# kivicode/TensorHive-Fixed

Hardware: AMD Instinct MI355X
Metric: llama3_8b_bf16_ddp_train_tokens_per_sec (higher is better)
Workload: dtype bf16; 1 GPU; model=Llama-3-8B, global_batch=8, micro_batch=8, grad_accum=1, seq_len=4096, parallelism=dp1, optimizer=AdamW (fp32 master, fused flat kernel, clip 1.0), zero=0, attention=hip, gemm_table=True, gemm_table_kind=gemm_gfx950_t32768.csv

## Files before the change

tensorhive_fixed_amd/models/llama3.py:

```python
from __future__ import annotations

import math
import os
from dataclasses import dataclass

import torch
from torch import nn

from ..ops.attention import qkv_attention
from ..ops.cross_entropy import linear_cross_entropy
from ..ops.embedding import embedding
from ..ops.linear import linear
from ..ops.mlp import gate_up_swiglu
from ..ops.rmsnorm import rmsnorm, rmsnorm_add_fork, rmsnorm_fork
from ..ops.swiglu import swiglu


@dataclass
class LlamaConfig:
    vocab_size: int = 128256
    dim: int = 4096
    n_layers: int = 32
    n_heads: int = 32
    n_kv_heads: int = 8
    ffn_dim: int = 14336
    rope_theta: float = 500000.0
    norm_eps: float = 1e-5
    max_seq_len: int = 8192
    ce_chunk: int = 4096

    @property
    def head_dim(self) -> int:
        return self.dim // self.n_heads

    @classmethod
    def llama3_8b(cls) -> "LlamaConfig":
        return cls(ce_chunk=int(os.environ.get("TH_CE_CHUNK", "4096")))

    @classmethod
    def tiny(cls) -> "LlamaConfig":
        return cls(vocab_size=512, dim=256, n_layers=2, n_heads=2, n_kv_heads=1, ffn_dim=512,
                   max_seq_len=512, ce_chunk=64)

    @classmethod
    def named(cls, name: str) -> "LlamaConfig":
        table = {"llama3-8b": cls.llama3_8b, "llama3_8b": cls.llama3_8b, "tiny": cls.tiny,
                 "llama3-1b-shape": lambda: cls(dim=2048, n_layers=16, n_heads=16, n_kv_heads=4,
                                                ffn_dim=8192)}
        return table[name.lower()]()

    def num_params(self) -> int:
        d, f, v, L = self.dim, self.ffn_dim, self.vocab_size, self.n_layers
        kv = self.n_kv_heads * self.head_dim
        per_layer = d * (d + 2 * kv) + d * d + 2 * f * d + f * d + 2 * d
        return v * d * 2 + L * per_layer + d

    def flops_per_token(self, seq_len: int) -> float:
        n_mat = self.num_params() - self.vocab_size * self.dim
        attn = 2 * 2 * self.n_layers * seq_len * self.dim / 2
        return 6 * n_mat + 3 * attn


WGRAD_NT = set(filter(None, os.environ.get("TH_WGRAD_NT_LAYERS", "w13").split(",")))
WGRAD_TN = set(filter(None, os.environ.get("TH_WGRAD_TN_LAYERS", "wqkv,wo,w2").split(",")))
_FORK = os.environ.get("TH_RMSNORM_FORK", "1") == "1"


ADD_NORM = _FORK and os.environ.get("TH_ADD_NORM", "1") == "1"


def _norm(x, w, eps):
    if _FORK:
        return rmsnorm_fork(x, w, eps)
    return rmsnorm(x, w, eps), x


class LlamaBlock(nn.Module):
    def __init__(self, cfg: LlamaConfig, device, dtype):
        super().__init__()
        d, hd = cfg.dim, cfg.head_dim
        qkv_out = (cfg.n_heads + 2 * cfg.n_kv_heads) * hd
        self.cfg = cfg
        self.attn_norm = nn.Parameter(torch.ones(d, device=device, dtype=dtype))
        self.wqkv = nn.Parameter(torch.empty(qkv_out, d, device=device, dtype=dtype))
        self.wo = nn.Parameter(torch.empty(d, cfg.n_heads * hd, device=device, dtype=dtype))
        self.ffn_norm = nn.Parameter(torch.ones(d, device=device, dtype=dtype))
        self.w13 = nn.Parameter(torch.empty(2 * cfg.ffn_dim, d, device=device, dtype=dtype))
        self.w2 = nn.Parameter(torch.empty(d, cfg.ffn_dim, device=device, dtype=dtype))

    def forward(self, x: torch.Tensor, B: int, S: int, pending: torch.Tensor | None = None):
        c = self.cfg
        if pending is not None:
            h, x = rmsnorm_add_fork(pending, x, self.attn_norm, c.norm_eps)
        else:
            h, x = _norm(x, self.attn_norm, c.norm_eps)
        qkv = linear(h, self.wqkv, wgrad_nt="wqkv" in WGRAD_NT, wgrad_tn="wqkv" in WGRAD_TN)
        o = qkv_attention(qkv, B, S, c.n_heads, c.n_kv_heads, c.head_dim, c.rope_theta)
        if ADD_NORM:
            y = linear(o, self.wo, wgrad_nt="wo" in WGRAD_NT, wgrad_tn="wo" in WGRAD_TN)
            h, x = rmsnorm_add_fork(y, x, self.ffn_norm, c.norm_eps)
        else:
            x = linear(o, self.wo, residual=x, wgrad_nt="wo" in WGRAD_NT, wgrad_tn="wo" in WGRAD_TN)
            h, x = _norm(x, self.ffn_norm, c.norm_eps)
        if "w13" in WGRAD_NT:
            a = gate_up_swiglu(h, self.w13)
        else:
            a = swiglu(linear(h, self.w13))
        if ADD_NORM:
            return linear(a, self.w2, wgrad_nt="w2" in WGRAD_NT, wgrad_tn="w2" in WGRAD_TN), x
        return linear(a, self.w2, residual=x, wgrad_nt="w2" in WGRAD_NT, wgrad_tn="w2" in WGRAD_TN)


class Llama(nn.Module):
    def __init__(self, cfg: LlamaConfig, device="cpu", dtype=torch.bfloat16, seed: int = 0):
        super().__init__()
        self.cfg = cfg
        self.tok_emb = nn.Parameter(torch.empty(cfg.vocab_size, cfg.dim, device=device, dtype=dtype))
        self.layers = nn.ModuleList([LlamaBlock(cfg, device, dtype) for _ in range(cfg.n_layers)])
        self.norm = nn.Parameter(torch.ones(cfg.dim, device=device, dtype=dtype))
        self.lm_head = nn.Parameter(torch.empty(cfg.vocab_size, cfg.dim, device=device, dtype=dtype))
        self.param_gate = None
        self.reset_parameters(seed)

    @torch.no_grad()
    def reset_parameters(self, seed: int = 0) -> None:
        g = torch.Generator(device=self.tok_emb.device)
        g.manual_seed(seed)
        std = 0.02
        out_std = std / math.sqrt(2 * self.cfg.n_layers)
        self.tok_emb.normal_(0, std, generator=g)
        self.lm_head.normal_(0, std, generator=g)
        for blk in self.layers:
            blk.wqkv.normal_(0, std, generator=g)
            blk.w13.normal_(0, std, generator=g)
            blk.wo.normal_(0, out_std, generator=g)
            blk.w2.normal_(0, out_std, generator=g)

    def params_in_backward_order(self) -> list[tuple[str, nn.Parameter, bool]]:
        out = [("lm_head", self.lm_head, True), ("norm", self.norm, False)]
        for i in reversed(range(len(self.layers))):
            b = self.layers[i]
            out += [(f"layers.{i}.w2", b.w2, True), (f"layers.{i}.w13", b.w13, True),
                    (f"layers.{i}.ffn_norm", b.ffn_norm, False), (f"layers.{i}.wo", b.wo, True),
                    (f"layers.{i}.wqkv", b.wqkv, True), (f"layers.{i}.attn_norm", b.attn_norm, False)]
        out.append(("tok_emb", self.tok_emb, True))
        return out

    def hidden(self, tokens: torch.Tensor) -> torch.Tensor:
        B, S = tokens.shape
        gate = self.param_gate
        if gate is not None:
            gate(self.tok_emb)
        x = embedding(tokens, self.tok_emb).view(B * S, self.cfg.dim)
        pending = None
        for blk in self.layers:
            if gate is not None:
                gate(blk.attn_norm, blk.wqkv, blk.wo, blk.ffn_norm, blk.w13, blk.w2)
            if ADD_NORM:
                pending, x = blk(x, B, S, pending)
            else:
                x = blk(x, B, S)
        if gate is not None:
            gate(self.norm, self.lm_head)
        if pending is not None:
            return rmsnorm_add_fork(pending, x, self.norm, self.cfg.norm_eps)[0]
        return rmsnorm(x, self.norm, self.cfg.norm_eps)

    def forward(self, tokens: torch.Tensor, targets: torch.Tensor | None = None,
                n_valid: int | None = None) -> torch.Tensor:
        h = self.hidden(tokens)
        if targets is None:
            return h
        return linear_cross_entropy(h, self.lm_head, targets.reshape(-1), self.cfg.ce_chunk,
                                    n_valid=n_valid)

    @torch.no_grad()
    def logits(self, tokens: torch.Tensor) -> torch.Tensor:
        return torch.mm(self.hidden(tokens), self.lm_head.t()).view(*tokens.shape, -1)
```

tensorhive_fixed_amd/ops/_lib.py:

```python
from __future__ import annotations

import ctypes as C
import os
import threading
from pathlib import Path

import torch

_HERE = Path(__file__).resolve().parent
_LIB_PATH = Path(os.environ.get("TH_KERNEL_LIB", _HERE / "libthk.so"))
_lock = threading.Lock()
_lib: C.CDLL | None = None

P = C.c_void_p
I = C.c_int
L = C.c_long
F = C.c_float

_SIGS: dict[str, list] = {
    "th_rmsnorm_fwd": [P, P, P, P, I, I, F, P],
    "th_rmsnorm_add_fwd": [P, P, P, P, P, P, I, I, F, P],
    "th_rmsnorm_bwd": [P, P, P, P, P, P, P, I, I, I, I, P, P],
    "th_swiglu_fwd": [P, P, L, I, P],
    "th_swiglu_bwd": [P, P, P, L, I, P],
    "th_swiglu_bwd_t": [P, P, P, P, L, I, P],
    "th_rope_inplace": [P, P, P, L, I, I, I, I, F, P],
    "th_sumsq_bf16": [P, L, P, P, I, P],
    "th_adamw_step": [P, P, P, P, P, L, F, F, F, F, F, I, F, P, F, P],
    "th_adamw_step_f32g": [P, P, P, P, P, L, F, F, F, F, F, I, F, P, F, P],
    "th_sumsq_f32": [P, L, P, P, I, P],
    "th_ce_fwd_bwd": [P, L, P, P, P, L, I, F, I, P],
    "th_flash_attn_fwd": [P, P, P, P, P, I, I, I, I, I, I, L, L, L, L, F, I, P],
    "th_flash_attn_bwd": [P, P, P, P, P, P, P, P, P, P, P, I, I, I, I, I, I, L, L, L, L, F, I, P],
    "th_flash_attn_bwd_rope": [P, P, P, P, P, P, P, P, P, P, I, I, I, I, I, I, L, L, L, L, F, P, P, I, P],
    "th_embedding_bwd": [P, P, P, P, L, I, I, P],
    "th_transpose_bf16": [P, P, L, L, L, I, P],
    "th_gemm_tn": [P, L, P, L, P, L, I, I, I, I, I, I, P, L, I, P],
    "th_comm_emu_launch": [P, P, L, L, L, L, P, I, L, I, P, P],
    "th_comm_emu_stop": [P, I, P],
}


def library_path() -> Path:
    return _LIB_PATH


def load(build_if_missing: bool = False) -> C.CDLL:
    global _lib
    if _lib is not None:
        return _lib
    with _lock:
        if _lib is not None:
            return _lib
        if not _LIB_PATH.exists() and build_if_missing:
            from . import build as _build

            _build.build()
        if not _LIB_PATH.exists():
            raise RuntimeError(
                f"gfx950 kernel library {_LIB_PATH} is missing: run "
                "`python -m tensorhive_fixed_amd.ops.build` (no eager fallback on GPU)")
        if "TH_KERNEL_LIB" not in os.environ:
            from . import build as _build

            if _build.stamp_exists() and not _build.is_up_to_date():
                if build_if_missing:
                    _build.build()
                else:
                    raise RuntimeError(f"{_LIB_PATH} was built from different sources than ops/csrc: rebuild "
                                       "with `python -m tensorhive_fixed_amd.ops.build`")
        lib = C.CDLL(str(_LIB_PATH))
        for name, argtypes in _SIGS.items():
            fn = getattr(lib, name, None)
            if fn is None:
                continue
            fn.argtypes = argtypes
            fn.restype = C.c_int
        _lib = lib
        return lib


def available() -> bool:
    try:
        load()
        return True
    except (RuntimeError, OSError):
        return False


def stream_ptr(device: torch.device | None = None) -> int:
    return torch.cuda.current_stream(device).cuda_stream


def ptr(t: torch.Tensor | None) -> int | None:
    return None if t is None else t.data_ptr()


def call(name: str, *args) -> None:
    fn = getattr(load(), name, None)
    if fn is None:
        raise RuntimeError(f"kernel entry point {name} not present in {_LIB_PATH}")
    rc = fn(*args)
    if rc != 0:
        raise RuntimeError(f"{name} failed with code {rc} ({'bad shape' if rc < 0 else 'hipError'})")
```

tensorhive_fixed_amd/ops/csrc/swiglu.hip:

```cpp
#include "th_common.h"

__device__ __forceinline__ float sigmoidf_(float g) { return 1.f / (1.f + __expf(-g)); }

__global__ __launch_bounds__(256) void swiglu_fwd_kernel(const ushort* __restrict__ gu,
                                                         ushort* __restrict__ out, long T, int F) {
  const int cpr = F >> 3;
  for (long row = blockIdx.x; row < T; row += gridDim.x) {
    const ushort* g_row = gu + row * 2 * F;
    ushort* o_row = out + row * F;
    for (int c = threadIdx.x; c < cpr; c += blockDim.x) {
      const ushort8 g = *reinterpret_cast<const ushort8*>(g_row + c * 8);
      const ushort8 u = *reinterpret_cast<const ushort8*>(g_row + F + c * 8);
      ushort8 o;
#pragma unroll
      for (int j = 0; j < 8; ++j) {
        const float gf = bf2f(g[j]);
        o[j] = f2bf(gf * sigmoidf_(gf) * bf2f(u[j]));
      }
      *reinterpret_cast<ushort8*>(o_row + c * 8) = o;
    }
  }
}

__global__ __launch_bounds__(256) void swiglu_bwd_kernel(const ushort* __restrict__ dout,
                                                         const ushort* __restrict__ gu,
                                                         ushort* __restrict__ dgu, long T, int F) {
  const int cpr = F >> 3;
  for (long row = blockIdx.x; row < T; row += gridDim.x) {
    for (int c = threadIdx.x; c < cpr; c += blockDim.x) {
      const ushort8 g = *reinterpret_cast<const ushort8*>(gu + row * 2 * F + c * 8);
      const ushort8 u = *reinterpret_cast<const ushort8*>(gu + row * 2 * F + F + c * 8);
      const ushort8 d = *reinterpret_cast<const ushort8*>(dout + row * F + c * 8);
      ushort8 dg, du;
#pragma unroll
      for (int j = 0; j < 8; ++j) {
        const float gf = bf2f(g[j]), uf = bf2f(u[j]), df = bf2f(d[j]);
        const float sg = sigmoidf_(gf);
        const float silu = gf * sg;
        du[j] = f2bf(df * silu);
        dg[j] = f2bf(df * uf * sg * (1.f + gf * (1.f - sg)));
      }
      *reinterpret_cast<ushort8*>(dgu + row * 2 * F + c * 8) = dg;
      *reinterpret_cast<ushort8*>(dgu + row * 2 * F + F + c * 8) = du;
    }
  }
}

constexpr int ST_R = 128, ST_C = 64;

__device__ __forceinline__ int st_swz(int r) { return 2 * (((r >> 1) & 1) | (((r >> 3) & 1) << 1)); }
__device__ __forceinline__ int st_off(int r, int chunk) { return r * 128 + ((chunk ^ st_swz(r)) << 4); }

typedef short i16x4s __attribute__((ext_vector_type(4)));
#define ST_LDS __attribute__((address_space(3)))

__global__ __launch_bounds__(256) void swiglu_bwd_t_kernel(const ushort* __restrict__ dout,
                                                           const ushort* __restrict__ gu,
                                                           ushort* __restrict__ dgu,
                                                           ushort* __restrict__ dguT, long T, int F) {
  __shared__ __attribute__((aligned(16))) char tile[2 * ST_R * 128];
  const int tid = threadIdx.x;
  const long ntc = F / ST_C;
  const long r0 = (blockIdx.x / ntc) * ST_R, c0 = (blockIdx.x % ntc) * ST_C;
  const int lch = tid & 7, lc = lch * 8;
  ushort8 g[4], u[4], d[4];
#pragma unroll
  for (int i = 0; i < 4; ++i) {
    const long row = r0 + (tid >> 3) + 32 * i;
    const long rr = row < T ? row : T - 1;
    g[i] = *reinterpret_cast<const ushort8*>(gu + rr * 2 * F + c0 + lc);
    u[i] = *reinterpret_cast<const ushort8*>(gu + rr * 2 * F + F + c0 + lc);
    d[i] = *reinterpret_cast<const ushort8*>(dout + rr * F + c0 + lc);
  }
#pragma unroll
  for (int i = 0; i < 4; ++i) {
    const int lr = (tid >> 3) + 32 * i;
    const long row = r0 + lr;
    ushort8 dg, du;
#pragma unroll
    for (int j = 0; j < 8; ++j) {
      const float gf = bf2f(g[i][j]), uf = bf2f(u[i][j]), df = bf2f(d[i][j]);
      const float sg = sigmoidf_(gf);
      du[j] = f2bf(df * gf * sg);
      dg[j] = f2bf(df * uf * sg * (1.f + gf * (1.f - sg)));
    }
    if (row < T) {
      *reinterpret_cast<ushort8*>(dgu + row * 2 * F + c0 + lc) = dg;
      *reinterpret_cast<ushort8*>(dgu + row * 2 * F + F + c0 + lc) = du;
    }
    *reinterpret_cast<ushort8*>(tile + st_off(lr, lch)) = dg;
    *reinterpret_cast<ushort8*>(tile + ST_R * 128 + st_off(lr, lch)) = du;
  }
  __syncthreads();
  const int lane = tid & 63, w = tid >> 6, grp = lane >> 4, i16 = lane & 15, q = i16 >> 2, p = i16 & 3;
#pragma unroll
  for (int k = 0; k < 8; ++k) {
    const int step = w * 8 + k;
    const int half = step >> 4, fb = (step >> 2) & 3, tg0 = (step & 3) * 32;
    const int rbase = tg0 + 8 * grp;
    const int col = fb * 16 + 4 * p;
    const char* base = tile + half * ST_R * 128 + ((col & 7) << 1);
    const int ch = col >> 3;
    const i16x4s lo = __builtin_amdgcn_ds_read_tr16_b64_v4i16((ST_LDS i16x4s*)(base + st_off(rbase + q, ch)));
    const i16x4s hi = __builtin_amdgcn_ds_read_tr16_b64_v4i16((ST_LDS i16x4s*)(base + st_off(rbase + 4 + q, ch)));
    ushort8 o;
#pragma unroll
    for (int e = 0; e < 4; ++e) {
      o[e] = (ushort)lo[e];
      o[4 + e] = (ushort)hi[e];
    }
    const long feat = (long)half * F + c0 + fb * 16 + i16;
    const long tok = r0 + rbase;
    if (tok < T) *reinterpret_cast<ushort8*>(dguT + feat * T + tok) = o;
  }
}

static unsigned grid_for(long rows) {
  long g = rows;
  if (g > 4096) g = 4096;
  if (g < 1) g = 1;
  return (unsigned)g;
}

extern "C" int th_swiglu_fwd(const void* gu, void* out, long T, int F, hipStream_t s) {
  if (F % 8 != 0 || T <= 0) return -1;
  swiglu_fwd_kernel<<<grid_for(T), 256, 0, s>>>((const ushort*)gu, (ushort*)out, T, F);
  TH_CHECK_LAUNCH();
}

extern "C" int th_swiglu_bwd(const void* dout, const void* gu, void* dgu, long T, int F,
                             hipStream_t s) {
  if (F % 8 != 0 || T <= 0) return -1;
  swiglu_bwd_kernel<<<grid_for(T), 256, 0, s>>>((const ushort*)dout, (const ushort*)gu,
                                                          (ushort*)dgu, T, F);
  TH_CHECK_LAUNCH();
}

extern "C" int th_swiglu_bwd_t(const void* dout, const void* gu, void* dgu, void* dguT, long T, int F,
                               hipStream_t s) {
  if (F % ST_C != 0 || T <= 0 || T % 8 != 0) return -1;
  const long tiles = ((T + ST_R - 1) / ST_R) * (F / ST_C);
  if (tiles > 0x7fffffffL) return -2;
  swiglu_bwd_t_kernel<<<(unsigned)tiles, 256, 0, s>>>((const ushort*)dout, (const ushort*)gu, (ushort*)dgu,
                                                      (ushort*)dguT, T, F);
  TH_CHECK_LAUNCH();
}
```

tensorhive_fixed_amd/ops/mlp.py:

```python
from __future__ import annotations

import os

import torch

from . import _lib
from ._grad import deliver, mm_into, nt_into, nt_mm
from .gemm_tn import gemm_tn_, supported as _tn_supported
from .linear import _DGRAD_NT, linear, tn_into
from .swiglu import swiglu, swiglu_reference
from .transpose import transpose


_W13_TN = os.environ.get("TH_W13_WGRAD_TN", "1") == "1"


class _GateUpSwiGLU(torch.autograd.Function):
    @staticmethod
    def forward(ctx, h: torch.Tensor, w13: torch.Tensor):
        h2 = h.reshape(-1, h.shape[-1])
        if not h2.is_contiguous():
            h2 = h2.contiguous()
        gu = nt_mm(h2, w13) if h2.is_cuda else torch.mm(h2, w13.t())
        T, F2 = gu.shape
        F = F2 // 2
        if gu.is_cuda:
            a = torch.empty((T, F), device=gu.device, dtype=gu.dtype)
            _lib.call("th_swiglu_fwd", gu.data_ptr(), a.data_ptr(), T, F, _lib.stream_ptr(gu.device))
        else:
            a = swiglu_reference(gu)
        ctx.save_for_backward(h2, w13, gu)
        ctx.hshape = h.shape
        return a.view(*h.shape[:-1], F)

    @staticmethod
    def backward(ctx, da: torch.Tensor):
        h2, w13, gu = ctx.saved_tensors
        T, F2 = gu.shape
        F = F2 // 2
        d2 = da.reshape(T, F)
        if not d2.is_contiguous():
            d2 = d2.contiguous()
        if gu.is_cuda and _W13_TN and _tn_supported(F2, h2.shape[1], T):
            dgu = torch.empty_like(gu)
            _lib.call("th_swiglu_bwd", d2.data_ptr(), gu.data_ptr(), dgu.data_ptr(), T, F, _lib.stream_ptr(gu.device))
            dh = nt_mm(dgu, transpose(w13)) if _DGRAD_NT else torch.mm(dgu, w13)
            gw = deliver(w13, tn_into(dgu, h2),
                         lambda: gemm_tn_(dgu, h2, torch.empty(w13.shape, device=gu.device, dtype=gu.dtype)))
            del dgu
        elif gu.is_cuda:
            dgu = torch.empty_like(gu)
            dguT = torch.empty((F2, T), device=gu.device, dtype=gu.dtype)
            _lib.call("th_swiglu_bwd_t", d2.data_ptr(), gu.data_ptr(), dgu.data_ptr(), dguT.data_ptr(), T, F,
                      _lib.stream_ptr(gu.device))
            dh = nt_mm(dgu, transpose(w13)) if _DGRAD_NT else torch.mm(dgu, w13)
            del dgu
            hT = transpose(h2)
            gw = deliver(w13, nt_into(dguT, hT), lambda: torch.mm(dguT, hT.t()))
        else:
            g, u = gu.float().chunk(2, dim=-1)
            s = torch.sigmoid(g)
            df = d2.float()
            dgu = torch.cat([df * u * s * (1 + g * (1 - s)), df * g * s], dim=-1).to(gu.dtype)
            dh = torch.mm(dgu, w13)
            gw = deliver(w13, mm_into(dgu.t(), h2), lambda: torch.mm(dgu.t(), h2))
        return dh.view(ctx.hshape), gw


def gate_up_swiglu(h: torch.Tensor, w13: torch.Tensor) -> torch.Tensor:
    F = w13.shape[0] // 2
    if h.is_cuda and (F % 64 or h.numel() // h.shape[-1] % 8):
        return swiglu(linear(h, w13, wgrad_nt=True))
    return _GateUpSwiGLU.apply(h, w13)
```

Before: 26670 tokens/s.

## Fuse MLP down-proj dgrad GEMM with SwiGLU backward in custom HIP kernel

Adds a custom 256x256 NT GEMM kernel for gfx950 whose epilogue applies the SwiGLU backward directly to the down-projection dgrad tile. It reads gate/up activations and writes dgu without materialising the intermediate dA tensor. The MLP forward and backward are wrapped in one autograd function that saves `a` and `gu`. This removes a full read and write of the T×F activation gradient and a separate elementwise launch. The cost is keeping `a` saved for backward, which adds memory, and relying on a hand-tuned kernel that may be slower than the table-tuned library GEMM.

After: 26810 tokens/s (median of 6 runs). Within noise of the previous version (+0.5%).

```diff
diff --git a/tensorhive_fixed_amd/models/llama3.py b/tensorhive_fixed_amd/models/llama3.py
--- a/tensorhive_fixed_amd/models/llama3.py
+++ b/tensorhive_fixed_amd/models/llama3.py
@@ -11,7 +11,7 @@
 from ..ops.cross_entropy import linear_cross_entropy
 from ..ops.embedding import embedding
 from ..ops.linear import linear
-from ..ops.mlp import gate_up_swiglu
+from ..ops.mlp import gate_up_swiglu, mlp_swiglu
 from ..ops.rmsnorm import rmsnorm, rmsnorm_add_fork, rmsnorm_fork
 from ..ops.swiglu import swiglu
 
@@ -102,6 +102,8 @@
         else:
             x = linear(o, self.wo, residual=x, wgrad_nt="wo" in WGRAD_NT, wgrad_tn="wo" in WGRAD_TN)
             h, x = _norm(x, self.ffn_norm, c.norm_eps)
+        if ADD_NORM and "w13" in WGRAD_NT and "w2" in WGRAD_TN and "w2" not in WGRAD_NT:
+            return mlp_swiglu(h, self.w13, self.w2), x
         if "w13" in WGRAD_NT:
             a = gate_up_swiglu(h, self.w13)
         else:
diff --git a/tensorhive_fixed_amd/ops/_lib.py b/tensorhive_fixed_amd/ops/_lib.py
--- a/tensorhive_fixed_amd/ops/_lib.py
+++ b/tensorhive_fixed_amd/ops/_lib.py
@@ -36,6 +36,7 @@
     "th_embedding_bwd": [P, P, P, P, L, I, I, P],
     "th_transpose_bf16": [P, P, L, L, L, I, P],
     "th_gemm_tn": [P, L, P, L, P, L, I, I, I, I, I, I, P, L, I, P],
+    "th_gemm_nt_mlp": [I, P, L, P, L, P, L, P, L, I, I, I, I, P],
     "th_comm_emu_launch": [P, P, L, L, L, L, P, I, L, I, P, P],
     "th_comm_emu_stop": [P, I, P],
 }
diff --git a/tensorhive_fixed_amd/ops/csrc/gemm_nt.hip b/tensorhive_fixed_amd/ops/csrc/gemm_nt.hip
--- /dev/null
+++ b/tensorhive_fixed_amd/ops/csrc/gemm_nt.hip
@@ -0,0 +1,273 @@
+#include "th_common.h"
+#include "swiglu_math.h"
+
+typedef __bf16 bf16x8 __attribute__((ext_vector_type(8)));
+typedef float f32x4 __attribute__((ext_vector_type(4)));
+typedef int i32x4 __attribute__((ext_vector_type(4)));
+#define LDS_AS __attribute__((address_space(3)))
+
+#ifndef TH_NT_GM
+#define TH_NT_GM 8
+#endif
+
+namespace {
+constexpr int BM = 256, BN = 256, BK = 64;
+constexpr int IMG = BM * BK * 2;
+constexpr int EPI_PLAIN = 0, EPI_BWD = 1;
+constexpr int PA0 = 22, PAS = 4, PB0 = 52, PBS = 5;
+
+__device__ __forceinline__ int xcd_remap(int bid, int nwg) {
+  const int xcd = bid & 7, q = nwg >> 3, r = nwg & 7;
+  return (xcd < r ? xcd * (q + 1) : r * (q + 1) + (xcd - r) * q) + (bid >> 3);
+}
+
+template <int I, int N, typename F>
+__device__ __forceinline__ void static_for_nt(F&& f) {
+  if constexpr (I < N) {
+    f(std::integral_constant<int, I>{});
+    static_for_nt<I + 1, N>(f);
+  }
+}
+
+__device__ __forceinline__ bf16x8 lds_rd(const char LDS_AS* p) { return *reinterpret_cast<const bf16x8 LDS_AS*>(p); }
+}
+
+template <int EPI>
+__global__ __launch_bounds__(256, 1) void gemm_nt_hb_kernel(const ushort* __restrict__ A, long lda,
+                                                          const ushort* __restrict__ B, long ldb,
+                                                          ushort* __restrict__ C, long ldc, ushort* X, long ldx, int M,
+                                                          int nN, int K, int F, int GM) {
+  __shared__ __attribute__((aligned(1024))) char smem_raw[4 * IMG];
+  const char LDS_AS* smem = (const char LDS_AS*)smem_raw;
+  const int nM = M / BM;
+  const int L = xcd_remap(blockIdx.x, gridDim.x);
+  const int per_band = GM * nN;
+  const int band = L / per_band;
+  const int first_m = band * GM;
+  const int gm = min(GM, nM - first_m);
+  const int in_band = L % per_band;
+  const int tm = first_m + in_band % gm;
+  const int tn = in_band / gm;
+  const long m0 = (long)tm * BM;
+  const long n0 = (long)tn * BN;
+
+  const int lane = threadIdx.x & 63;
+  const int w = __builtin_amdgcn_readfirstlane(threadIdx.x >> 6);
+  const int wm = w >> 1, wn = w & 1;
+  const int r16 = lane & 15, g = lane >> 4;
+  auto img = [](int op, int st) { return op * 2 * IMG + st * IMG; };
+  int rda[2], rdb[2];
+#pragma unroll
+  for (int ks = 0; ks < 2; ++ks) {
+    const int o = r16 * 128 + (((4 * ks + g) ^ (r16 >> 1)) << 4);
+    rda[ks] = wm * (128 * 128) + o;
+    rdb[ks] = img(1, 0) + wn * (128 * 128) + o;
+  }
+  auto rd_frag = [&](int st, int f, int ks) -> bf16x8 {
+    return f < 8 ? lds_rd(smem + rda[ks] + st * IMG + f * 2048) : lds_rd(smem + rdb[ks] + st * IMG + (f - 8) * 2048);
+  };
+  const int dma_row = w * 64;
+  const ushort* ga = A + (m0 + dma_row) * lda;
+  const ushort* gb = B + (n0 + dma_row) * ldb;
+  unsigned va[2], vb[2];
+#pragma unroll
+  for (int par = 0; par < 2; ++par) {
+    const int rr = lane >> 3, slot = lane & 7;
+    const int chunk = slot ^ (4 * par + (lane >> 4));
+    va[par] = (unsigned)(2 * ((long)rr * lda + 8 * chunk));
+    vb[par] = (unsigned)(2 * ((long)rr * ldb + 8 * chunk));
+  }
+  const unsigned lds0 = (unsigned)(uintptr_t)(char LDS_AS*)smem_raw;
+  const unsigned lds_w = __builtin_amdgcn_readfirstlane(lds0 + (unsigned)dma_row * 128u);
+  const unsigned sa_step = (unsigned)(2L * 8 * lda), sb_step = (unsigned)(2L * 8 * ldb);
+  auto piece = [&](int op, int p, int kt, int st) {
+    const ushort* base = (op == 0 ? ga : gb) + (long)kt * BK;
+    const __amdgpu_buffer_rsrc_t r = __builtin_amdgcn_make_buffer_rsrc((void*)base, 0, 0x7fffffff, 0x00020000);
+    const unsigned soff = (unsigned)p * (op == 0 ? sa_step : sb_step);
+    const unsigned voff = op == 0 ? va[p & 1] : vb[p & 1];
+    const unsigned lb = __builtin_amdgcn_readfirstlane(lds_w + img(op, st) + p * 1024);
+    asm volatile("s_mov_b32 m0, %0\n\ts_nop 0\n\tbuffer_load_dwordx4 %1, %2, %3 offen lds"
+                 :: "s"(lb), "v"(voff), "s"(r), "s"(soff) : "memory", "m0");
+  };
+  auto piece_load_w = [&](int op, int p, unsigned long long base) {
+    const i32x4 r = {(int)(unsigned)base, (int)(unsigned)(base >> 32), 0x7fffffff, 0x00020000};
+    const unsigned soff = (unsigned)p * (op == 0 ? sa_step : sb_step);
+    const unsigned voff = op == 0 ? va[p & 1] : vb[p & 1];
+    asm volatile("buffer_load_dwordx4 %0, %1, %2 offen lds" :: "v"(voff), "s"(r), "s"(soff) : "memory", "m0");
+  };
+
+  f32x4 acc[8][8];
+#pragma unroll
+  for (int i = 0; i < 8; ++i)
+#pragma unroll
+    for (int j = 0; j < 8; ++j) acc[i][j] = f32x4(0.f);
+#pragma unroll
+  for (int i = 0; i < 8; ++i)
+#pragma unroll
+    for (int j = 0; j < 8; ++j) asm volatile("" : "+a"(acc[i][j]));
+  asm volatile("s_nop 4" ::);
+
+  const int nt = K / BK;
+#pragma unroll
+  for (int p = 0; p < 8; ++p) piece(0, p, 0, 0);
+#pragma unroll
+  for (int p = 0; p < 8; ++p) piece(1, p, 0, 0);
+  const int kt1 = min(1, nt - 1);
+#pragma unroll
+  for (int p = 0; p < 8; ++p) piece(0, p, kt1, 1);
+#pragma unroll
+  for (int p = 0; p < 8; ++p) piece(1, p, kt1, 1);
+  asm volatile("s_waitcnt vmcnt(16)\n\ts_barrier" ::: "memory");
+  bf16x8 xa[8], xb[8], ya[8], yb[8];
+#pragma unroll
+  for (int f = 0; f < 8; ++f) {
+    xa[f] = rd_frag(0, f, 0);
+    xb[f] = rd_frag(0, 8 + f, 0);
+  }
+  auto mf = [&](f32x4& c, const bf16x8& b, const bf16x8& a) {
+    asm volatile("v_mfma_f32_16x16x32_bf16 %0, %1, %2, %0" : "+a"(c) : "v"(b), "v"(a));
+  };
+  unsigned long long ra2 = (unsigned long long)(uintptr_t)(ga + (long)min(2, nt - 1) * BK);
+  unsigned long long rb2 = (unsigned long long)(uintptr_t)(gb + (long)min(2, nt - 1) * BK);
+  auto ktile = [&](auto stc) {
+    constexpr int ST = decltype(stc)::value;
+    static_for_nt<0, 128>([&](auto mc) {
+      constexpr int m = decltype(mc)::value;
+      constexpr int mm = m & 63, i = mm >> 3, j = mm & 7;
+      static_assert(PA0 > 20 && PA0 + 7 * PAS < PB0 && PB0 > 44 && PB0 + 7 * PBS < 88, "NT DMA slots");
+      constexpr bool pa = m >= PA0 && m < PA0 + 8 * PAS && (m - PA0) % PAS == 0;
+      constexpr bool pb = m >= PB0 && m < PB0 + 8 * PBS && (m - PB0) % PBS == 0;
+      constexpr int pi = pa ? (m - PA0) / PAS : (pb ? (m - PB0) / PBS : 0);
+      constexpr int poff = (pb ? 2 * IMG : 0) + ST * IMG + 1024 * pi;
+      if constexpr (pa || pb) asm volatile("s_add_i32 m0, %0, %1" :: "s"(lds_w), "n"(poff) : "m0");
+      if constexpr (m < 64)
+        mf(acc[i][j], xb[j], xa[i]);
+      else
+        mf(acc[i][j], yb[j], ya[i]);
+      if constexpr (m < 16 && !(m & 1)) ya[m >> 1] = rd_frag(ST, m >> 1, 1);
+      if constexpr (m == 20) asm volatile("s_waitcnt lgkmcnt(0)\n\ts_barrier" ::: "memory");
+      if constexpr (pa) piece_load_w(0, pi, ra2);
+      if constexpr (m >= 23 && m <= 37 && (m & 1)) yb[(m - 23) >> 1] = rd_frag(ST, 8 + ((m - 23) >> 1), 1);
+      if constexpr (m == 44) asm volatile("s_waitcnt lgkmcnt(0)\n\ts_barrier" ::: "memory");
+      if constexpr (pb) piece_load_w(1, pi, rb2);
+      if constexpr (m == 88) asm volatile("s_waitcnt vmcnt(16)\n\ts_barrier" ::: "memory");
+      if constexpr (m >= 90 && m <= 120 && !(m & 1)) {
+        constexpr int ord[16] = {0, 8, 9, 10, 11, 12, 13, 14, 15, 1, 2, 3, 4, 5, 6, 7};
+        constexpr int f = ord[(m - 90) >> 1];
+        if constexpr (f < 8) xa[f] = rd_frag(ST ^ 1, f, 0);
+        else xb[f - 8] = rd_frag(ST ^ 1, f, 0);
+      }
+      __builtin_amdgcn_sched_barrier(0);
+    });
+  };
+  int t = 0;
+  auto advance = [&]() {
+    const unsigned step = t + 3 < nt ? (unsigned)(BK * 2) : 0u;
+    ra2 += step;
+    rb2 += step;
+    ++t;
+  };
+  for (; t + 1 < nt;) {
+    ktile(std::integral_constant<int, 0>{});
+    advance();
+    ktile(std::integral_constant<int, 1>{});
+    advance();
+  }
+  if (t < nt) {
+    ktile(std::integral_constant<int, 0>{});
+    advance();
+  }
+  asm volatile("s_waitcnt vmcnt(0) lgkmcnt(0)\n\ts_barrier\n\ts_nop 15\n\ts_nop 15" ::: "memory");
+#pragma unroll
+  for (int i = 0; i < 8; ++i)
+#pragma unroll
+    for (int j = 0; j < 8; ++j) asm volatile("" : "+a"(acc[i][j]));
+
+  const long brow0 = m0 + wm * 128, bcol0 = n0 + wn * 128;
+  ushort8 gq[2][8], uq[2][8];
+  auto bwd_load = [&](int grp) {
+#pragma unroll
+    for (int k = 0; k < 8; ++k) {
+      const ushort* gp = X + (brow0 + 4 * (8 * grp + k) + g) * ldx + bcol0 + 8 * r16;
+      gq[grp & 1][k] = *reinterpret_cast<const ushort8*>(gp);
+      uq[grp & 1][k] = *reinterpret_cast<const ushort8*>(gp + F);
+    }
+  };
+  if constexpr (EPI == EPI_BWD) {
+    bwd_load(0);
+    __builtin_amdgcn_sched_barrier(0);
+  }
+  char LDS_AS* ep = (char LDS_AS*)smem_raw + w * 32768;
+#pragma unroll
+  for (int i = 0; i < 8; ++i) {
+#pragma unroll
+    for (int j = 0; j < 8; ++j) {
+      const f32x4 v = acc[i][j];
+      ushort4v o;
+#pragma unroll
+      for (int e = 0; e < 4; ++e) o[e] = f2bf(v[e]);
+      const int row = 16 * i + r16;
+      const int blk = (2 * j + (g >> 1)) ^ r16;
+      *reinterpret_cast<ushort4v LDS_AS*>(ep + row * 256 + blk * 16 + (g & 1) * 8) = o;
+    }
+  }
+  if constexpr (EPI == EPI_PLAIN) {
+    const long crow0 = m0 + wm * 128, ccol0 = n0 + wn * 128;
+#pragma unroll
+    for (int q = 0; q < 32; ++q) {
+      const int row = 4 * q + g;
+      const ushort8 v = *reinterpret_cast<const ushort8 LDS_AS*>(ep + row * 256 + ((r16 ^ (row & 15)) << 4));
+      *reinterpret_cast<ushort8*>(C + (crow0 + row) * ldc + ccol0 + 8 * r16) = v;
+    }
+  } else {
+#pragma unroll
+    for (int grp = 0; grp < 4; ++grp) {
+      if (grp + 1 < 4) bwd_load(grp + 1);
+      __builtin_amdgcn_sched_barrier(0);
+#pragma unroll
+      for (int k = 0; k < 8; ++k) {
+        const int row = 4 * (8 * grp + k) + g;
+        const ushort8 gv = gq[grp & 1][k], uv = uq[grp & 1][k];
+        const ushort8 dv = *reinterpret_cast<const ushort8 LDS_AS*>(ep + row * 256 + ((r16 ^ (row & 15)) << 4));
+        ushort8 dg, du;
+#pragma unroll
+        for (int e = 0; e < 8; ++e) {
+          ushort dge, due;
+          swiglu_bwd_elem(gv[e], uv[e], dv[e], dge, due);
+          dg[e] = dge;
+          du[e] = due;
+        }
+        ushort* cp = C + (brow0 + row) * ldc + bcol0 + 8 * r16;
+        *reinterpret_cast<ushort8*>(cp) = dg;
+        *reinterpret_cast<ushort8*>(cp + F) = du;
+      }
+      __builtin_amdgcn_sched_barrier(0);
+    }
+  }
+}
+
+extern "C" int th_gemm_nt_mlp(int mode, const void* A, long lda, const void* B, long ldb, void* C, long ldc, void* X,
+                              long ldx, int M, int F, int K, int gm, hipStream_t s) {
+  if (mode < 0 || mode > 1 || M <= 0 || F <= 0 || K < 128 || M % BM || F % BN || K % BK) return -1;
+  const long cw = mode == 0 ? F : 2L * F;
+  if (lda < K || ldb < K || ldc < cw || lda % 8 || ldb % 8 || ldc % 8) return -1;
+  if (((uintptr_t)A | (uintptr_t)B | (uintptr_t)C) & 15) return -1;
+  if (mode != 0) {
+    if (X == nullptr || ((uintptr_t)X & 15) || ldx % 8 || ldx < 2L * F) return -1;
+  }
+  if (gm < 0 || gm > 64) return -1;
+  if (2L * 64 * max(lda, ldb) + 128 >= (1L << 31)) return -1;
+  const int nN = F / BN;
+  const long grid = (long)(M / BM) * nN;
+  if (grid > 0x7fffffffL) return -2;
+  const int GM = gm ? gm : TH_NT_GM;
+#define TH_NT_LAUNCH(EPI)                                                                                          \
+  gemm_nt_hb_kernel<EPI><<<(unsigned)grid, 256, 0, s>>>((const ushort*)A, lda, (const ushort*)B, ldb, (ushort*)C, ldc, \
+                                                        (ushort*)X, ldx, M, nN, K, F, GM)
+  if (mode == 1)
+    TH_NT_LAUNCH(EPI_BWD);
+  else
+    TH_NT_LAUNCH(EPI_PLAIN);
+#undef TH_NT_LAUNCH
+  TH_CHECK_LAUNCH();
+}
diff --git a/tensorhive_fixed_amd/ops/csrc/swiglu.hip b/tensorhive_fixed_amd/ops/csrc/swiglu.hip
--- a/tensorhive_fixed_amd/ops/csrc/swiglu.hip
+++ b/tensorhive_fixed_amd/ops/csrc/swiglu.hip
@@ -1,6 +1,5 @@
 #include "th_common.h"
-
-__device__ __forceinline__ float sigmoidf_(float g) { return 1.f / (1.f + __expf(-g)); }
+#include "swiglu_math.h"
 
 __global__ __launch_bounds__(256) void swiglu_fwd_kernel(const ushort* __restrict__ gu,
                                                          ushort* __restrict__ out, long T, int F) {
@@ -13,10 +12,7 @@
       const ushort8 u = *reinterpret_cast<const ushort8*>(g_row + F + c * 8);
       ushort8 o;
 #pragma unroll
-      for (int j = 0; j < 8; ++j) {
-        const float gf = bf2f(g[j]);
-        o[j] = f2bf(gf * sigmoidf_(gf) * bf2f(u[j]));
-      }
+      for (int j = 0; j < 8; ++j) o[j] = swiglu_fwd_elem(g[j], u[j]);
       *reinterpret_cast<ushort8*>(o_row + c * 8) = o;
     }
   }
@@ -34,11 +30,10 @@
       ushort8 dg, du;
 #pragma unroll
       for (int j = 0; j < 8; ++j) {
-        const float gf = bf2f(g[j]), uf = bf2f(u[j]), df = bf2f(d[j]);
-        const float sg = sigmoidf_(gf);
-        const float silu = gf * sg;
-        du[j] = f2bf(df * silu);
-        dg[j] = f2bf(df * uf * sg * (1.f + gf * (1.f - sg)));
+        ushort dgj, duj;
+        swiglu_bwd_elem(g[j], u[j], d[j], dgj, duj);
+        dg[j] = dgj;
+        du[j] = duj;
       }
       *reinterpret_cast<ushort8*>(dgu + row * 2 * F + c * 8) = dg;
       *reinterpret_cast<ushort8*>(dgu + row * 2 * F + F + c * 8) = du;
diff --git a/tensorhive_fixed_amd/ops/csrc/swiglu_math.h b/tensorhive_fixed_amd/ops/csrc/swiglu_math.h
--- /dev/null
+++ b/tensorhive_fixed_amd/ops/csrc/swiglu_math.h
@@ -0,0 +1,17 @@
+#pragma once
+#include "th_common.h"
+
+__device__ __forceinline__ float sigmoidf_(float g) { return 1.f / (1.f + __expf(-g)); }
+
+__device__ __forceinline__ ushort swiglu_fwd_elem(ushort g, ushort u) {
+  const float gf = bf2f(g);
+  return f2bf(gf * sigmoidf_(gf) * bf2f(u));
+}
+
+__device__ __forceinline__ void swiglu_bwd_elem(ushort g, ushort u, ushort d, ushort& dg, ushort& du) {
+  const float gf = bf2f(g), uf = bf2f(u), df = bf2f(d);
+  const float sg = sigmoidf_(gf);
+  const float silu = gf * sg;
+  du = f2bf(df * silu);
+  dg = f2bf(df * uf * sg * (1.f + gf * (1.f - sg)));
+}
diff --git a/tensorhive_fixed_amd/ops/gemm_nt.py b/tensorhive_fixed_amd/ops/gemm_nt.py
--- /dev/null
+++ b/tensorhive_fixed_amd/ops/gemm_nt.py
@@ -0,0 +1,54 @@
+from __future__ import annotations
+
+import torch
+
+from . import _lib
+
+PLAIN, BWD = 0, 1
+_TM, _TK = 256, 64
+
+
+def supported(mode: int, t: int, f: int, k: int) -> bool:
+    if mode not in (PLAIN, BWD) or t <= 0 or f <= 0:
+        return False
+    return t % _TM == 0 and f % 256 == 0 and k % _TK == 0 and k >= 2 * _TK
+
+
+def _row_major_ok(*ts: torch.Tensor) -> bool:
+    return all(x.is_cuda and x.dtype == torch.bfloat16 and x.dim() == 2 and x.stride(1) == 1
+               and x.stride(0) % 8 == 0 and x.data_ptr() % 16 == 0 for x in ts)
+
+
+def usable(mode: int, a: torch.Tensor, b: torch.Tensor, *rest: torch.Tensor) -> bool:
+    t, k = a.shape
+    return (b.shape[1] == k and supported(mode, t, b.shape[0], k) and _row_major_ok(a, b, *rest)
+            and 128 * max(a.stride(0), b.stride(0)) + 128 < (1 << 31))
+
+
+def default_band(mode: int) -> int:
+    return 4 if mode == BWD else 0
+
+
+def _launch(mode, a, b, c, x, f, band):
+    if band is None:
+        band = default_band(mode)
+    if not 0 <= int(band) <= 64:
+        raise ValueError(f"gemm_nt: band {band} not in 0..64")
+    _lib.call("th_gemm_nt_mlp", mode, a.data_ptr(), a.stride(0), b.data_ptr(), b.stride(0), c.data_ptr(), c.stride(0),
+              None if x is None else x.data_ptr(), 0 if x is None else x.stride(0), a.shape[0], f, a.shape[1],
+              int(band), _lib.stream_ptr(a.device))
+
+
+def nt_plain_(a: torch.Tensor, b: torch.Tensor, out: torch.Tensor, band: int | None = None) -> torch.Tensor:
+    if tuple(out.shape) != (a.shape[0], b.shape[0]) or not usable(PLAIN, a, b, out):
+        raise ValueError(f"nt_plain_: unsupported {tuple(a.shape)} x {tuple(b.shape)} -> {tuple(out.shape)}")
+    _launch(PLAIN, a, b, out, None, b.shape[0], band)
+    return out
+
+
+def down_dgrad_swiglu_(dy: torch.Tensor, w2t: torch.Tensor, gu: torch.Tensor, dgu: torch.Tensor,
+                       band: int | None = None) -> None:
+    t, f = dy.shape[0], w2t.shape[0]
+    if tuple(gu.shape) != (t, 2 * f) or tuple(dgu.shape) != (t, 2 * f) or not usable(BWD, dy, w2t, dgu, gu):
+        raise ValueError(f"down_dgrad_swiglu_: unsupported {tuple(dy.shape)} x {tuple(w2t.shape)}")
+    _launch(BWD, dy, w2t, dgu, gu, f, band)
diff --git a/tensorhive_fixed_amd/ops/mlp.py b/tensorhive_fixed_amd/ops/mlp.py
--- a/tensorhive_fixed_amd/ops/mlp.py
+++ b/tensorhive_fixed_amd/ops/mlp.py
@@ -4,10 +4,10 @@
 
 import torch
 
-from . import _lib
+from . import _lib, gemm_nt
 from ._grad import deliver, mm_into, nt_into, nt_mm
 from .gemm_tn import gemm_tn_, supported as _tn_supported
-from .linear import _DGRAD_NT, linear, tn_into
+from .linear import _DGRAD_NT, _WGRAD_TN, linear, tn_into
 from .swiglu import swiglu, swiglu_reference
 from .transpose import transpose
 
@@ -72,3 +72,71 @@
     if h.is_cuda and (F % 64 or h.numel() // h.shape[-1] % 8):
         return swiglu(linear(h, w13, wgrad_nt=True))
     return _GateUpSwiGLU.apply(h, w13)
+
+
+_FUSED_MODES = {"0": False, "bwd": True, "1": True}
+
+
+def _fused_mode(value: str, what: str) -> bool:
+    if value == "fwd":
+        raise ValueError(f"{what}=fwd: the forward fusion measured slower in the step and is not in the tree "
+                         "(profiles/r07_mlp_fused/)")
+    if value not in _FUSED_MODES:
+        raise ValueError(f"{what}={value!r}: expected one of {sorted(_FUSED_MODES)}")
+    return _FUSED_MODES[value]
+
+
+_FUSED = os.environ.get("TH_MLP_FUSED", "1")
+_fused_mode(_FUSED, "TH_MLP_FUSED")
+
+
+def mlp_fusions(mode: str, t: int, d: int, f: int) -> bool:
+    if not _fused_mode(mode, "mlp_fusions: mode"):
+        return False
+    if not (_W13_TN and _WGRAD_TN and _DGRAD_NT and _tn_supported(2 * f, d, t) and _tn_supported(d, f, t)):
+        return False
+    return gemm_nt.supported(gemm_nt.BWD, t, f, d)
+
+
+class _MlpSwiGLU(torch.autograd.Function):
+
+    @staticmethod
+    def forward(ctx, h: torch.Tensor, w13: torch.Tensor, w2: torch.Tensor):
+        h2 = h.reshape(-1, h.shape[-1])
+        if not h2.is_contiguous():
+            h2 = h2.contiguous()
+        T, F = h2.shape[0], w13.shape[0] // 2
+        gu = nt_mm(h2, w13)
+        a = torch.empty((T, F), device=h2.device, dtype=h2.dtype)
+        _lib.call("th_swiglu_fwd", gu.data_ptr(), a.data_ptr(), T, F, _lib.stream_ptr(gu.device))
+        y = nt_mm(a, w2)
+        ctx.save_for_backward(h2, w13, gu, a, w2)
+        ctx.hshape = h.shape
+        return y.view(*h.shape[:-1], w2.shape[0])
+
+    @staticmethod
+    def backward(ctx, dy: torch.Tensor):
+        h2, w13, gu, a, w2 = ctx.saved_tensors
+        T = gu.shape[0]
+        dy2 = dy.reshape(T, w2.shape[0])
+        if not dy2.is_contiguous():
+            dy2 = dy2.contiguous()
+        w2t = transpose(w2)
+        dgu = torch.empty_like(gu)
+        gemm_nt.down_dgrad_swiglu_(dy2, w2t, gu, dgu)
+        del w2t
+        gw2 = deliver(w2, tn_into(dy2, a), lambda: torch.mm(dy2.t(), a))
+        dh = nt_mm(dgu, transpose(w13))
+        gw13 = deliver(w13, tn_into(dgu, h2),
+                       lambda: gemm_tn_(dgu, h2, torch.empty(w13.shape, device=gu.device, dtype=gu.dtype)))
+        return dh.view(ctx.hshape), gw13, gw2
+
+
+def mlp_swiglu(h: torch.Tensor, w13: torch.Tensor, w2: torch.Tensor, fused: str | None = None) -> torch.Tensor:
+    mode = _FUSED if fused is None else str(fused)
+    want = _fused_mode(mode, "mlp_swiglu: fused")
+    if (want and h.is_cuda and h.dtype == w13.dtype == w2.dtype == torch.bfloat16
+            and w13.is_contiguous() and w2.is_contiguous()
+            and mlp_fusions(mode, h.numel() // h.shape[-1], h.shape[-1], w13.shape[0] // 2)):
+        return _MlpSwiGLU.apply(h, w13, w2)
+    return linear(gate_up_swiglu(h, w13), w2, wgrad_tn=True)
```
